# GuanLab/seekmer

Measured on AMD Instinct MI355X. Metric: paired reads/sec mapped+quantified, higher is better.
Workload: dtype u64+f64; 1 GPU; configs[1]: synthetic ~190k-tx index (stand-in for ENSEMBL GRCh38 cDNA), 10000000 2x100bp synthetic pairs per GPU, map+classes+EM to the reference stop rule; transcripts=190402, kmer_slots=134217728, units_per_gpu=10000000, read_len=100, paired=True, classes=851072, class_map_rows=4208693, parallelism=reads sharded x1, RCCL all-reduce f64[T] per EM step, rccl_ranks=0

## Files before the change

### seekmer_amd/csrc/skm_abi.hip

```cpp
#include "../../include/seekmer_hip.h"
#include "skm_kernels.h"
#include "skm_pool.h"

#include <dlfcn.h>
#include <algorithm>
#include <cstdarg>
#include <cstdio>
#include <cstdlib>
#include <cstring>
#include <chrono>
#include <condition_variable>
#include <atomic>
#include <deque>
#include <functional>
#include <map>
#include <memory>
#include <unordered_map>
#include <mutex>
#include <thread>
#include <numeric>
#include <string>
#include <utility>
#include <vector>

// ... 230 lines not shown
    PoolPinned pinned;
    std::mutex mu;
    int64_t n_tx = 0, n_classes = 0, n_ids = 0, n_rows = 0;
    DBuf<int64_t> cls_offset, row_start, tx_row;
    DBuf<int32_t> ids, tx_cls, row_tx, perm;
    DBuf<double> cls_count, cls_count_saved, inner, row_sum;
    DBuf<double> eff_len, x0, x1, acc, part_max;
    DBuf<unsigned int> part_flags, arrivals;
    DBuf<unsigned long long> ctl, cum;
    DBuf<unsigned int> tile_total;
    DBuf<double> x_start, boot_out;
    struct Batch {
        DBuf<double> cls_count, inner, row_sum, x0, x1, part_max;
        DBuf<unsigned int> part_flags;
        DBuf<unsigned long long> ctl, mgr;
        DBuf<double> counts_all;
        DBuf<double> totals;
        DBuf<int64_t> iters;
    } batch;
    struct Tiles {
        DBuf<int64_t> tile_tx, tile_cls, cls_pair, tx_pair;
        DBuf<int32_t> tx_list, cls_list, tx_label, tx_tile, cls_tile;
        DBuf<uint16_t> cls_tx, tx_cls;
        DBuf<double> snap, step_max;
        DBuf<unsigned int> step_flags;
        struct Residual {
            int64_t n_classes = 0, n_ids = 0, n_rows = 0;
            DBuf<int64_t> cls_offset, row_start, tx_row;
            DBuf<int32_t> ids, cls_src, row_tx, tx_cls;
            DBuf<double> cls_count, inner, row_sum;
            bool built = false;
        } residual;
        bool built = false;
        int64_t n_tiles = 0, n_oversize = 0;
    } tiles;
    double n_total = 0;
    bool n_total_reduced = false;
    void *comm = nullptr;
    int rank = 0, world = 1;
    double t_em_ns = 0, iters_total = 0, launches = 0;
};

struct skm_comm {
    int device = 0;
    void *comm = nullptr;
    int rank = 0, world = 1;
};

// ... 2341 lines not shown
    q->n_classes = n_classes;
    q->n_ids = n_ids;
    HIP_TRY(pool_stream_acquire(q->stream.out()));
    for (auto &e : q->ev) HIP_TRY(pool_event_acquire(e.out(), true));
    for (auto &e : q->chunk_ev) HIP_TRY(pool_event_acquire(e.out(), false));
    HIP_TRY(pool_pinned_acquire((void **)q->pinned.out()));
    const size_t C = (size_t)std::max<int64_t>(n_classes, 1), M = (size_t)std::max<int64_t>(n_ids, 1);
    const size_t T = (size_t)std::max<int64_t>(n_tx, 1);
    const size_t R = (size_t)quant_rows_upper_bound(n_tx, n_ids);
    SKM_TRY(q->cls_offset.ensure(C + 1));
    SKM_TRY(q->cls_count.ensure(C));
    SKM_TRY(q->inner.ensure(C));
    SKM_TRY(q->ids.ensure(M));
    SKM_TRY(q->perm.ensure(C));
    SKM_TRY(q->tx_cls.ensure(M));
    SKM_TRY(q->tx_row.ensure(T + 1));
    SKM_TRY(q->row_start.ensure(R + 1));
    SKM_TRY(q->row_tx.ensure(R));
    SKM_TRY(q->row_sum.ensure(R));
    SKM_TRY(q->eff_len.ensure(T));
    SKM_TRY(q->x0.ensure(T));
    SKM_TRY(q->x1.ensure(T));
    SKM_TRY(q->acc.ensure(T));
    SKM_TRY(q->ctl.ensure(16));
    SKM_TRY(q->part_max.ensure(EM_FINAL_BLOCKS));
    SKM_TRY(q->part_flags.ensure(EM_FINAL_BLOCKS));
    SKM_TRY(q->arrivals.ensure(T));
    HIP_TRY(hipMemsetAsync(q->arrivals.p, 0, T * sizeof(unsigned int), q->stream));
    if (em_tiles_possible(several_ranks)) {
        auto &t = q->tiles;
        SKM_TRY(t.tile_tx.ensure(T + 2)); SKM_TRY(t.tile_cls.ensure(T + 2));
        SKM_TRY(t.cls_pair.ensure(C + 1)); SKM_TRY(t.tx_pair.ensure(T + 1));
        SKM_TRY(t.tx_list.ensure(T)); SKM_TRY(t.cls_list.ensure(C));
        SKM_TRY(t.tx_label.ensure(T)); SKM_TRY(t.tx_tile.ensure(T)); SKM_TRY(t.cls_tile.ensure(C));
        SKM_TRY(t.cls_tx.ensure(M)); SKM_TRY(t.tx_cls.ensure(M));
    }
    STALE_CHECK("quant_alloc exit");
    return SKM_OK;
}

QuantBuild quant_build_view(skm_quant *q)
{
    QuantBuild b{};
    b.n_tx = q->n_tx;
    b.n_classes = q->n_classes;
    b.n_ids = q->n_ids;
    b.cls_offset = q->cls_offset.p;
// ... 8 lines not shown
        auto &t = q->tiles;
        b.tile_tx = t.tile_tx.p; b.tile_cls = t.tile_cls.p;
        b.tx_list = t.tx_list.p; b.cls_list = t.cls_list.p;
        b.cls_pair = t.cls_pair.p; b.tx_pair = t.tx_pair.p;
        b.tile_cls_tx = t.cls_tx.p; b.tile_tx_cls = t.tx_cls.p;
        b.tx_label = t.tx_label.p; b.tx_tile = t.tx_tile.p; b.cls_tile = t.cls_tile.p;
    }
    return b;
}

int quant_finish_setup(skm_quant *q, const ClassTable *table, int64_t units_seen = -1)
{
    STALE_CHECK("quant_finish_setup");
    QuantBuild b = quant_build_view(q);
    b.first_seen_bound = units_seen > 0 ? units_seen : 0;
    const int64_t rows = quant_setup(table, b, q->perm.p, q->stream);
    if (rows < 0) return fail(SKM_ERR_HIP, "building the class views failed (%lld): %s", (long long)rows, quant_setup_failure());
    q->n_rows = rows;
    if (b.tile_tx) {
        q->tiles.built = true;
        q->tiles.n_tiles = b.tile_info[0];
        q->tiles.n_oversize = b.tile_info[1];
        if (q->tiles.n_tiles > 0) {
            SKM_TRY(q->tiles.step_max.ensure((size_t)(EM_CHUNK_MAX * q->tiles.n_tiles)));
            SKM_TRY(q->tiles.step_flags.ensure((size_t)(EM_CHUNK_MAX * q->tiles.n_tiles)));
            SKM_TRY(q->tiles.snap.ensure((size_t)EM_CHUNK_MAX * (size_t)q->n_tx));
        }
        if (q->tiles.n_oversize > 0 && q->tiles.n_tiles > 0) {
            auto &r = q->tiles.residual;
            int64_t counts[3] = {0, 0, 0};
            if (quant_residual_count(b, counts, q->stream))
                return fail(SKM_ERR_HIP, "sizing the residual EM problem failed: %s", quant_setup_failure());
            r.n_classes = counts[0]; r.n_ids = counts[1]; r.n_rows = counts[2];
            SKM_TRY(r.cls_offset.ensure((size_t)r.n_classes + 1)); SKM_TRY(r.ids.ensure((size_t)std::max<int64_t>(r.n_ids, 1)));
            SKM_TRY(r.cls_src.ensure((size_t)std::max<int64_t>(r.n_classes, 1)));
            SKM_TRY(r.row_start.ensure((size_t)r.n_rows + 1)); SKM_TRY(r.row_tx.ensure((size_t)std::max<int64_t>(r.n_rows, 1)));
            SKM_TRY(r.tx_cls.ensure((size_t)std::max<int64_t>(r.n_ids, 1))); SKM_TRY(r.tx_row.ensure((size_t)q->n_tx + 1));
            SKM_TRY(r.cls_count.ensure((size_t)std::max<int64_t>(r.n_classes, 1)));
            SKM_TRY(r.inner.ensure((size_t)std::max<int64_t>(r.n_classes, 1)));
            SKM_TRY(r.row_sum.ensure((size_t)std::max<int64_t>(r.n_rows, 1)));
            QuantResidual out{};
            out.n_classes = r.n_classes; out.n_ids = r.n_ids; out.n_rows = r.n_rows;
            out.cls_offset = r.cls_offset.p; out.ids = r.ids.p; out.cls_src = r.cls_src.p;
            out.row_start = r.row_start.p; out.row_tx = r.row_tx.p; out.tx_cls = r.tx_cls.p; out.tx_row = r.tx_row.p;
            if (quant_residual_build(b, out, q->stream))
                return fail(SKM_ERR_HIP, "building the residual EM problem failed: %s", quant_setup_failure());
            r.built = true;
        }
// ... 98 lines not shown
        SKM_TRY(enqueue(slot));
        HIP_TRY(hipEventRecord(q->chunk_ev[slot], q->stream));
        return SKM_OK;
    };
    SKM_TRY(enqueue_chunk(0));
    for (int slot = 0;; slot ^= 1) {
        SKM_TRY(enqueue_chunk(slot ^ 1));
        HIP_TRY(hipEventSynchronize(q->chunk_ev[slot]));
        memcpy(words, q->pinned + 8 * slot, sizeof(words));
        if (stopped(words)) return SKM_OK;
    }
}
bool em_ctl_done(const unsigned long long *ctl) { return ctl[CTL_DONE] != 0; }

int em_run_tiles(skm_quant *q, const EmProblem &p, int64_t chunk, int64_t *iters_out)
{
    auto &t = q->tiles;
    EmTiles tl{};
    tl.n_tiles = t.n_tiles;
    tl.tile_tx = t.tile_tx.p; tl.tile_cls = t.tile_cls.p;
    tl.tx_list = t.tx_list.p; tl.cls_list = t.cls_list.p;
    tl.cls_pair = t.cls_pair.p; tl.tx_pair = t.tx_pair.p;
    tl.cls_tx = t.cls_tx.p; tl.tx_cls = t.tx_cls.p;
    tl.step_max = t.step_max.p; tl.step_flags = t.step_flags.p;
    tl.snap = t.snap.p;
    const bool mixed = t.n_oversize > 0;
    EmProblem pr = p;
    if (mixed) {
        auto &r = t.residual;
        pr.n_classes = r.n_classes; pr.n_rows = r.n_rows;
        pr.cls_offset = r.cls_offset.p; pr.ids = r.ids.p; pr.cls_count = r.cls_count.p; pr.inner = r.inner.p;
        pr.row_start = r.row_start.p; pr.row_tx = r.row_tx.p; pr.tx_cls = r.tx_cls.p; pr.tx_row = r.tx_row.p;
        pr.row_sum = r.row_sum.p;
        pr.fused = 1;
        pr.extra_max = t.step_max.p; pr.extra_flags = t.step_flags.p; pr.n_extra = t.n_tiles;
        launch_permute_f64(q->cls_count.p, r.cls_src.p, r.n_classes, r.cls_count.p, false, q->stream);
    }
    int64_t queued = 0;
    auto enqueue_chunk = [&](int slot) -> int {
        launch_em_local_chunk(p, tl, queued == 0 ? q->x0.p : t.snap.p + (chunk - 1) * q->n_tx, (int)chunk, queued * chunk, q->stream);
        if (mixed) {
            pr.extra_first = queued * chunk;
            for (int64_t i = 0, k = queued * chunk; i < chunk; ++i, ++k) {
                launch_em_inner(pr, (int)(k & 1), i > 0, k, q->stream);
                launch_em_rows_finalize(pr, (int)(k & 1), q->stream);
            }
            launch_em_decide(pr, (queued + 1) * chunk, q->stream);
            q->launches += 2 * chunk + 2;
        } else {
            launch_em_local_decide(p, tl, queued * chunk, (int)chunk, q->stream);
            q->launches += 2;
        }
        ++queued;
        HIP_TRY(hipGetLastError());
        HIP_TRY(hipMemcpyAsync(q->pinned + 8 * slot, q->ctl.p, 8 * sizeof(unsigned long long),
                               hipMemcpyDeviceToHost, q->stream));
        return SKM_OK;
    };
    unsigned long long ctl[8] = {0};
    SKM_TRY(em_run_chunks_ahead(q, ctl, enqueue_chunk, em_ctl_done));
    if (ctl[CTL_TILE_FAULT]) {
        HIP_TRY(hipStreamSynchronize(q->stream));
        return fail(SKM_ERR_STATE, "a component tile exceeds the tile capacity: the class views of this handle are damaged");
    }
    const int64_t steps = (int64_t)ctl[CTL_ITERS];
    HIP_TRY(hipEventRecord(q->ev[1], q->stream));
    HIP_TRY(hipEventSynchronize(q->ev[1]));
    float ms = 0;
    HIP_TRY(hipEventElapsedTime(&ms, q->ev[0], q->ev[1]));
    q->t_em_ns += ms * 1e6;
    q->iters_total += (double)steps;
    if (iters_out) *iters_out = steps;
    if (ctl[CTL_UNDEFINED]) return fail(SKM_ERR_UNDEFINED, "no abundance above x_floor: numpy raises on max() of an empty selection");
    return SKM_OK;
}

int em_run(skm_quant *q, double rel_tol, double x_floor, int64_t max_iters, int64_t fixed_iters,
           int64_t *iters_out, int64_t chunk_steps = 16)
{
    double n_total = q->n_total;
    if (q->comm && !q->n_total_reduced) {
        HIP_TRY(hipMemcpyAsync(q->acc.p, &n_total, 8, hipMemcpyHostToDevice, q->stream));
        NCCL_TRY(g_rccl.AllReduce(q->acc.p, q->acc.p, 1, NCCL_FLOAT64, NCCL_SUM, q->comm, q->stream));
        HIP_TRY(hipMemcpyAsync(&n_total, q->acc.p, 8, hipMemcpyDeviceToHost, q->stream));
        HIP_TRY(hipStreamSynchronize(q->stream));
    }
    EmProblem p = em_problem(q, rel_tol, x_floor, max_iters, fixed_iters);
    p.n_total = n_total;
    HIP_TRY(hipMemsetAsync(q->ctl.p, 0, 16 * 8, q->stream));
    int64_t k = 0;
    const int64_t chunk = fixed_iters > 0 ? std::min<int64_t>(fixed_iters, chunk_steps) : chunk_steps;
    HIP_TRY(hipEventRecord(q->ev[0], q->stream));
    if (em_uses_tiles(q) && chunk <= EM_CHUNK_MAX) return em_run_tiles(q, p, chunk, iters_out);
    static const bool unfused_rows = getenv("SKM_EM_UNFUSED") != nullptr;
    auto enqueue_chunk = [&](int slot) -> int {
        for (int64_t i = 0; i < chunk; ++i, ++k) {
            launch_em_inner(p, (int)(k & 1), i > 0, k, q->stream);
            if (q->comm) {
                if (unfused_rows) {
                    launch_em_rows(p, (int)(k & 1), q->stream);
                    launch_em_rows_to_acc(p, q->stream);
                } else {
                    launch_em_rows_acc(p, (int)(k & 1), q->stream);
                }
                NCCL_TRY(g_rccl.AllReduce(q->acc.p, q->acc.p, (size_t)q->n_tx, NCCL_FLOAT64, NCCL_SUM,
                                          q->comm, q->stream));
                launch_em_finalize(p, (int)(k & 1), true, q->stream);
            } else if (p.fused) {
                launch_em_rows_finalize(p, (int)(k & 1), q->stream);
            } else {
                launch_em_rows(p, (int)(k & 1), q->stream);
                launch_em_finalize(p, (int)(k & 1), false, q->stream);
// ... 210 lines not shown
    if (!q || !x || !l) return fail(SKM_ERR_ARG, "NULL argument");
    std::lock_guard<std::mutex> lock(q->mu);
    SKM_TRY(set_device(q->device));
    HIP_TRY(hipMemcpyAsync(q->x0.p, x, q->n_tx * 8, hipMemcpyHostToDevice, q->stream));
    HIP_TRY(hipMemcpyAsync(q->eff_len.p, l, q->n_tx * 8, hipMemcpyHostToDevice, q->stream));
    int64_t it = 0;
    SKM_TRY(em_run(q, rel_tol, x_floor, max_iters, fixed_iters, &it));
    HIP_TRY(hipMemcpy(x, (it & 1) ? q->x1.p : q->x0.p, q->n_tx * 8, hipMemcpyDeviceToHost));
    if (iters) *iters = it;
    return SKM_OK;
}

extern "C" int skm_quant_components(skm_quant *q, int64_t info[8], int32_t *tx_label, int32_t *tx_tile,
                                    int32_t *class_tile)
{
    if (!q || !info) return fail(SKM_ERR_ARG, "NULL argument");
    std::lock_guard<std::mutex> lock(q->mu);
    SKM_TRY(set_device(q->device));
    const auto &t = q->tiles;
    info[0] = t.built ? 1 : 0;
    info[1] = t.n_tiles;
    info[2] = t.n_oversize;
    info[3] = em_uses_tiles(q) ? 1 : 0;
    info[4] = EM_TILE_PAIRS; info[5] = EM_TILE_CLASSES; info[6] = EM_TILE_TX; info[7] = 0;
    if (!t.built) {
        if (tx_label || tx_tile || class_tile) return fail(SKM_ERR_ARG, "no component tiles were built for this handle");
        return SKM_OK;
    }
    HIP_TRY(hipStreamSynchronize(q->stream));
    if (tx_label) HIP_TRY(hipMemcpy(tx_label, t.tx_label.p, q->n_tx * 4, hipMemcpyDeviceToHost));
    if (tx_tile) HIP_TRY(hipMemcpy(tx_tile, t.tx_tile.p, q->n_tx * 4, hipMemcpyDeviceToHost));
    if (class_tile && q->n_classes) {
        std::vector<int32_t> tile(q->n_classes), perm(q->n_classes);
        HIP_TRY(hipMemcpy(tile.data(), t.cls_tile.p, q->n_classes * 4, hipMemcpyDeviceToHost));
        HIP_TRY(hipMemcpy(perm.data(), q->perm.p, q->n_classes * 4, hipMemcpyDeviceToHost));
        for (int64_t k = 0; k < q->n_classes; ++k) class_tile[perm[k]] = tile[k];
    }
    return SKM_OK;
}

extern "C" int skm_quant_set_counts(skm_quant *q, const double *class_counts)
{
    if (!q || (!class_counts && q->n_classes)) return fail(SKM_ERR_ARG, "NULL argument");
    std::lock_guard<std::mutex> lock(q->mu);
    SKM_TRY(set_device(q->device));
    const double total = np_sum_host(class_counts, q->n_classes);
    if (q->n_classes) {
// ... 845 lines not shown
```

### seekmer_amd/csrc/skm_em.hip

```cpp
#include "skm_em_core.h"

namespace skm {

__device__ bool em_evaluate(const EmProblem &p, int n_parts, int64_t steps_done, bool publish);

struct EmWholeTable {
    const EmProblem &p;
    __device__ __forceinline__ int64_t cls_first() const { return 0; }
    __device__ __forceinline__ int64_t cls_end() const { return p.n_classes; }
    __device__ __forceinline__ int64_t row_first() const { return 0; }
    __device__ __forceinline__ int64_t row_end() const { return p.n_rows; }
    __device__ __forceinline__ double n_total() const { return p.n_total; }
    __device__ __forceinline__ bool done() const { return p.ctl[CTL_DONE] != 0; }
    __device__ __forceinline__ bool judge(int eval_parts, int64_t steps_done) const { return em_evaluate(p, eval_parts, steps_done, true); }
    __device__ __forceinline__ int64_t part() const { return blockIdx.x; }
};

__global__ void __launch_bounds__(256)
em_inner_kernel(EmProblem p, int parity, int eval_parts, int64_t steps_done)
{
    em_inner_body(p, EmWholeTable{p}, parity, eval_parts > 0 && blockIdx.x == 0, eval_parts, steps_done, blockIdx.x * (int64_t)blockDim.x + threadIdx.x,
                  (int64_t)gridDim.x * blockDim.x);
}

// ... 110 lines not shown
    __shared__ uint16_t s_cls_tx[EM_TILE_PAIRS], s_tx_cls[EM_TILE_PAIRS];
    __shared__ uint16_t s_cls_off[EM_TILE_CLASSES + 1], s_tx_off[EM_TILE_TX + 1];
    const int64_t tile = blockIdx.x;
    const int64_t tx0 = tl.tile_tx[tile], cls0 = tl.tile_cls[tile];
    const int n_tx = (int)(tl.tile_tx[tile + 1] - tx0), n_cls = (int)(tl.tile_cls[tile + 1] - cls0);
    const int64_t cp0 = tl.cls_pair[cls0], tp0 = tl.tx_pair[tx0];
    const int n_pairs = (int)(tl.cls_pair[cls0 + n_cls] - cp0);
    if (n_tx > EM_TILE_TX || n_cls > EM_TILE_CLASSES || n_pairs > EM_TILE_PAIRS || n_tx < 0 || n_cls < 0 || n_pairs < 0) {
        if (threadIdx.x == 0) { p.ctl[CTL_TILE_FAULT] = 1; p.ctl[CTL_DONE] = 1; }
        return;
    }
    const int tid = threadIdx.x;
    if (p.ctl[CTL_DONE]) {
        const int64_t steps = (int64_t)p.ctl[CTL_ITERS], at = steps - 1 - (first_step - n_steps);
        if (p.ctl[CTL_TILE_FAULT] || first_step < n_steps || at < 0 || at >= n_steps) return;
        const double *__restrict__ from = tl.snap + at * p.n_tx;
        double *__restrict__ to = p.x[steps & 1];
        for (int i = tid; i < n_tx; i += 256) {
            const int32_t t = tl.tx_list[tx0 + i];
            to[t] = from[t];
        }
        return;
    }
    for (int j = tid; j < n_pairs; j += 256) {
        s_cls_tx[j] = tl.cls_tx[cp0 + j];
        s_tx_cls[j] = tl.tx_cls[tp0 + j];
    }
    for (int k = tid; k <= n_cls; k += 256) {
        s_cls_off[k] = (uint16_t)(tl.cls_pair[cls0 + k] - cp0);
        if (k < n_cls) s_count[k] = p.cls_count[tl.cls_list[cls0 + k]];
        if ((SKM_EM_TILE_EXPERIMENT & 1) && k < n_cls) s_inner[k] = 1.0;
    }
    for (int i = tid; i <= n_tx; i += 256) {
        s_tx_off[i] = (uint16_t)(tl.tx_pair[tx0 + i] - tp0);
        if (i < n_tx) {
            const int32_t t = tl.tx_list[tx0 + i];
            s_tx[i] = t;
            s_x[0][i] = x_in[t];
            s_eff[i] = p.eff_len[t];
        }
    }
    __syncthreads();
    const int sub = tid & 7, wave = tid >> 6;
    for (int step = 0; step < n_steps; ++step) {
        const double *x = s_x[step & 1];
        double *x_new = s_x[(step & 1) ^ 1];
// ... 35 lines not shown
                double a = 0.0;
                do {
                    const int row_end = min(begin + EM_ROW_CAP, end);
                    a += em_row_sum<false>(s_tx_cls, s_inner, begin, row_end, sub, xt);
                    begin = row_end;
                } while (begin < end);
                if (turn == sub) { my_a = a; my_xt = xt; my_i = i; }
            }
        }
        if (my_i >= 0) {
            const double v = em_new_abundance(my_a, s_eff[my_i], p.n_total);
            x_new[my_i] = v;
            tl.snap[step * p.n_tx + s_tx[my_i]] = v;
            em_note_change(v, my_xt, p.x_floor, local_max, flags);
        }
        em_wave_reduce<1>(local_max, flags);
        if ((tid & 63) == 0) { s_max[step][wave] = local_max; s_flags[step][wave] = flags; }
        __syncthreads();
    }
    if (tid < n_steps) {
        double m;
        unsigned int f;
        em_fold_waves(s_max[tid], s_flags[tid], 1, m, f);
        tl.step_max[tid * tl.n_tiles + tile] = m;
        tl.step_flags[tid * tl.n_tiles + tile] = f;
    }
}

__global__ void __launch_bounds__(64 * EM_CHUNK_MAX)
em_local_decide_kernel(EmProblem p, EmTiles tl, int64_t first_step, int n_steps)
{
    if (p.ctl[CTL_DONE]) return;
    __shared__ double s_max[EM_CHUNK_MAX];
    __shared__ unsigned int s_flags[EM_CHUNK_MAX];
    const int step = threadIdx.x >> 6, lane = threadIdx.x & 63;
    if (step < n_steps) {
        double m = 0.0;
        unsigned int f = 0;
        const double *__restrict__ step_max = tl.step_max + step * tl.n_tiles;
        const unsigned int *__restrict__ step_flags = tl.step_flags + step * tl.n_tiles;
        int64_t b = lane;
        for (; b + 7 * 64 < tl.n_tiles; b += 8 * 64) {
            double o[8];
            unsigned int g[8];
#pragma unroll
            for (int k = 0; k < 8; ++k) { o[k] = step_max[b + 64 * k]; g[k] = step_flags[b + 64 * k]; }
#pragma unroll
            for (int k = 0; k < 8; ++k) { m = o[k] > m ? o[k] : m; f |= g[k]; }
        }
        for (; b < tl.n_tiles; b += 64) {
            const double o = step_max[b];
            m = o > m ? o : m;
            f |= step_flags[b];
        }
        em_wave_reduce<1>(m, f);
        if (lane == 0) { s_max[step] = m; s_flags[step] = f; }
    }
    __syncthreads();
    if (threadIdx.x != 0) return;
    for (int s = 0; s < n_steps; ++s) {
        const int64_t steps_done = first_step + s + 1;
        const EmVerdict verdict = em_stop_rule(s_flags[s], s_max[s], p.rel_tol, steps_done, p.max_iters, p.fixed_iters);
        if (verdict.undefined) p.ctl[CTL_UNDEFINED] = 1;
        p.ctl[CTL_ITERS] = (unsigned long long)steps_done;
        p.ctl[CTL_DONE] = verdict.done ? 1ULL : 0ULL;
        if (verdict.done) break;
    }
}

__global__ void __launch_bounds__(256)
effective_lengths_kernel(const unsigned long long *__restrict__ fld,
                         const double *__restrict__ lengths, int64_t n_tx, double *__restrict__ out)
{
    fld += (int64_t)blockIdx.y * MAX_FRAGMENT_LENGTH;
    out += (int64_t)blockIdx.y * n_tx;
    __shared__ double p[MAX_FRAGMENT_LENGTH];
    __shared__ int bin[MAX_FRAGMENT_LENGTH];
    __shared__ unsigned long long counts[MAX_FRAGMENT_LENGTH];
    __shared__ unsigned long long part[4];
    __shared__ int n_bins;
    unsigned long long mine = 0;
    for (int i = threadIdx.x; i < MAX_FRAGMENT_LENGTH; i += blockDim.x) {
        counts[i] = fld[i];
        mine += counts[i];
    }
    for (int d = 32; d > 0; d >>= 1) mine += __shfl_xor(mine, d, 64);
    if ((threadIdx.x & 63) == 0) part[threadIdx.x >> 6] = mine;
    __syncthreads();
    const double total = (double)(long long)(part[0] + part[1] + part[2] + part[3]);
    if (threadIdx.x < 64) {
        int n = 0;
        for (int first = 0; first < MAX_FRAGMENT_LENGTH; first += 64) {
// ... 244 lines not shown

void launch_em_rows_finalize(const EmProblem &p, int parity, hipStream_t stream)
{
    hipLaunchKernelGGL(em_rows_finalize_kernel<false>, dim3((unsigned)em_final_blocks(p)), dim3(256), 0, stream, p, parity);
}

void launch_em_rows_acc(const EmProblem &p, int parity, hipStream_t stream)
{
    EmProblem fused = p;
    fused.fused = 1;
    hipLaunchKernelGGL(em_rows_finalize_kernel<true>, dim3((unsigned)em_final_blocks(fused)), dim3(256), 0, stream, p, parity);
}

void launch_em_local_chunk(const EmProblem &p, const EmTiles &tiles, const double *x_in, int n_steps, int64_t first_step,
                           hipStream_t stream)
{
    if (tiles.n_tiles <= 0 || n_steps <= 0) return;
    hipLaunchKernelGGL(em_local_chunk_kernel, dim3((unsigned)tiles.n_tiles), dim3(256), 0, stream, p, tiles, x_in,
                       std::min(n_steps, EM_CHUNK_MAX), first_step);
}

void launch_em_local_decide(const EmProblem &p, const EmTiles &tiles, int64_t first_step, int n_steps, hipStream_t stream)
{
    hipLaunchKernelGGL(em_local_decide_kernel, dim3(1), dim3(64 * EM_CHUNK_MAX), 0, stream, p, tiles, first_step,
                       std::min(n_steps, EM_CHUNK_MAX));
}

void launch_em_rows_to_acc(const EmProblem &p, hipStream_t stream)
{
    hipLaunchKernelGGL(em_rows_to_acc_kernel, dim3(chip_grid(p.n_tx, 256)), dim3(256), 0, stream, p);
}

void launch_em_finalize(const EmProblem &p, int parity, bool from_acc, hipStream_t stream)
{
    const int blocks = em_final_blocks(p);
    if (from_acc)
        hipLaunchKernelGGL(em_finalize_kernel<true>, dim3((unsigned)blocks), dim3(256), 0, stream, p, parity);
    else
        hipLaunchKernelGGL(em_finalize_kernel<false>, dim3((unsigned)blocks), dim3(256), 0, stream, p, parity);
}

constexpr int NP_MAX_LEAVES = 160;

__device__ __forceinline__ double np_leaf_sum(const double *a, int n)
{
    if (n < 8) {
        double r = 0.0;
// ... 289 lines not shown
```

### seekmer_amd/csrc/skm_kernels.h

```cpp
#pragma once
#include "skm_device.h"

namespace skm {

struct MapBatch {
    const uint32_t *records;
    int64_t n_units;
    int32_t words_per_read;
    int32_t record_words;
    int32_t paired;
    int32_t *workspace;
    int32_t *rec_unit;
    uint64_t *rec_key;
    unsigned long long *rec_tuple;
    int32_t keep_spans;
    int32_t *unit_begin, *unit_end;
    Coord *unit_anchor;
    int32_t *unit_entries;
    int64_t ids_capacity;
    unsigned long long *ids_cursor;
    unsigned long long *fld;
    unsigned long long *stats;
    int32_t vote[8];
};
// ... 143 lines not shown
    int fused;
    unsigned int *arrivals;
    const double *extra_max;
    const unsigned int *extra_flags;
    int64_t n_extra, extra_first;
};
enum { CTL_DONE = 0, CTL_ITERS = 1, CTL_UNDEFINED = 3, CTL_TILE_FAULT = 4 };
#ifndef SKM_EM_FINAL_BLOCKS
#define SKM_EM_FINAL_BLOCKS 2048
#endif
constexpr int EM_FINAL_BLOCKS = SKM_EM_FINAL_BLOCKS;
void launch_em_inner(const EmProblem &p, int parity, bool judge_previous, int64_t steps_done, hipStream_t stream);
void launch_em_decide(const EmProblem &p, int64_t steps_done, hipStream_t stream);
void launch_em_rows(const EmProblem &p, int parity, hipStream_t stream);
void launch_em_rows_finalize(const EmProblem &p, int parity, hipStream_t stream);
void launch_em_rows_acc(const EmProblem &p, int parity, hipStream_t stream);
void launch_em_rows_to_acc(const EmProblem &p, hipStream_t stream);
void launch_em_finalize(const EmProblem &p, int parity, bool from_acc, hipStream_t stream);
void launch_em_result(const unsigned long long *ctl, const double *x0, const double *x1, int64_t n, double *out,
                      hipStream_t stream);

constexpr int EM_TILE_PAIRS = 2048, EM_TILE_CLASSES = 512, EM_TILE_TX = 128;
#ifndef SKM_EM_TILE_SEGMENT
#define SKM_EM_TILE_SEGMENT 128
#endif
constexpr int EM_TILE_SEGMENT = SKM_EM_TILE_SEGMENT;
constexpr int EM_CHUNK_MAX = 16;
constexpr int EM_TILE_CLASS_BATCH = 4;
struct EmTiles {
    int64_t n_tiles;
    const int64_t *tile_tx;
    const int64_t *tile_cls;
    const int32_t *tx_list;
    const int32_t *cls_list;
    const int64_t *cls_pair;
    const int64_t *tx_pair;
    const uint16_t *cls_tx;
    const uint16_t *tx_cls;
    double *step_max;
    unsigned int *step_flags;
    double *snap;
};
void launch_em_local_chunk(const EmProblem &p, const EmTiles &tiles, const double *x_in, int n_steps, int64_t first_step,
                           hipStream_t stream);
void launch_em_local_decide(const EmProblem &p, const EmTiles &tiles, int64_t first_step, int n_steps, hipStream_t stream);

constexpr int EM_BATCH = 8;
struct EmBatchProblem {
    int64_t n_tx, n_classes, n_rows;
    const int64_t *cls_offset;
    const int32_t *ids;
    const int64_t *row_start;
    const int32_t *row_tx;
    const int32_t *tx_cls;
    const int64_t *tx_row;
    const double *eff_len;
    const double *cls_count;
    double *inner;
    double *row_sum;
    double *x[2];
    double *place_total;
    double rel_tol, x_floor;
    unsigned long long *ctl;
// ... 125 lines not shown
```

### seekmer_amd/csrc/skm_quant_setup.hip

```cpp
#include "skm_kernels.h"
#include "skm_pool.h"

#include <algorithm>
#include <cstdio>
#include <vector>

namespace skm {

namespace {

struct Scratch {
    hipStream_t stream;
    std::vector<void *> held;
    explicit Scratch(hipStream_t s) : stream(s) {}
    template <class T>
    T *alloc(size_t n)
    {
        void *p = nullptr;
        if (pool_alloc(&p, std::max<size_t>(n, 1) * sizeof(T)) != hipSuccess) return nullptr;
        held.push_back(p);
        return static_cast<T *>(p);
    }
    ~Scratch()
    {
// ... 705 lines not shown
__global__ void __launch_bounds__(256)
cc_classes_kernel(const int64_t *cls_offset, const int32_t *ids, int64_t n_classes, const int32_t *label,
                  int32_t *comp)
{
    const int lane = threadIdx.x & 63;
    const int64_t stride = (int64_t)gridDim.x * blockDim.x;
    for (int64_t c0 = blockIdx.x * (int64_t)blockDim.x + threadIdx.x - lane; c0 < n_classes; c0 += stride) {
        const int64_t c = c0 + lane;
        int32_t r = -1;
        if (c < n_classes) {
            const int64_t begin = cls_offset[c];
            r = label[begin < cls_offset[c + 1] ? ids[begin] : 0];
        }
        const int32_t before = __shfl_up(r, 1, 64);
        const unsigned long long heads = __ballot(lane == 0 || before != r);
        if (r >= 0 && ((heads >> lane) & 1ULL)) {
            const unsigned long long later = lane == 63 ? 0ULL : heads >> (lane + 1);
            const int run = later ? __ffsll((long long)later) : 64 - lane;
            atomicAdd(&comp[3 * (int64_t)r + 2], run);
        }
    }
}

__global__ void __launch_bounds__(256)
tile_pack_kernel(const int32_t *__restrict__ comp, int64_t n_tx, int64_t n_segments, int32_t *__restrict__ root_tile,
                 int64_t *__restrict__ seg_tiles, unsigned long long *__restrict__ oversize)
{
    for (int64_t g = blockIdx.x * (int64_t)blockDim.x + threadIdx.x; g < n_segments;
         g += (int64_t)gridDim.x * blockDim.x) {
        int tx = 0, pairs = 0, classes = 0, n = 0;
        const int64_t last = min(n_tx, (g + 1) * EM_TILE_SEGMENT);
        for (int64_t t0 = g * EM_TILE_SEGMENT; t0 < last; t0 += 8) {
            int size[24];
#pragma unroll
            for (int k = 0; k < 24; ++k) size[k] = 3 * t0 + k < 3 * n_tx ? comp[3 * t0 + k] : 0;
#pragma unroll
            for (int k = 0; k < 8; ++k) {
                const int64_t t = t0 + k;
                if (t >= last) break;
                const int c_tx = size[3 * k], c_pairs = size[3 * k + 1], c_classes = size[3 * k + 2];
                if (c_tx == 0) { root_tile[t] = -1; continue; }
                if (c_tx > EM_TILE_TX || c_pairs > EM_TILE_PAIRS || c_classes > EM_TILE_CLASSES) {
                    root_tile[t] = -2;
                    atomicAdd(oversize, 1ULL);
                    continue;
                }
                if (n == 0 || tx + c_tx > EM_TILE_TX || pairs + c_pairs > EM_TILE_PAIRS ||
                    classes + c_classes > EM_TILE_CLASSES) {
                    ++n;
                    tx = pairs = classes = 0;
                }
                tx += c_tx; pairs += c_pairs; classes += c_classes;
                root_tile[t] = n - 1;
            }
        }
        seg_tiles[g] = n;
    }
}

__global__ void __launch_bounds__(256)
tx_tile_kernel(const int32_t *label, const int32_t *root_tile, const int64_t *seg_base, int64_t n_tx,
               const int64_t *tx_row, const int64_t *row_start, int degree_bits, int32_t *tx_tile, int32_t *key)
{
    for (int64_t t = blockIdx.x * (int64_t)blockDim.x + threadIdx.x; t < n_tx;
         t += (int64_t)gridDim.x * blockDim.x) {
        const int32_t r = label[t], at = root_tile[r];
        const int32_t tile = at < 0 ? (int32_t)n_tx : (int32_t)(seg_base[r / EM_TILE_SEGMENT] + at);
        tx_tile[t] = tile;
        const int64_t turns = (row_start[tx_row[t + 1]] - row_start[tx_row[t]] + 7) >> 3;
        const int32_t longest = (1 << degree_bits) - 1;
        key[t] = (tile << degree_bits) | (longest - (int32_t)min(turns, (int64_t)longest));
    }
}

#ifndef SKM_EM_CLASS_ORDER
#define SKM_EM_CLASS_ORDER 1
#endif
__global__ void __launch_bounds__(256)
cls_tile_kernel(const int64_t *cls_offset, const int32_t *ids, int64_t n_classes, const int32_t *tx_tile,
                int length_bits, int32_t *cls_tile, int32_t *key)
{
// ... 73 lines not shown
    }
}

int build_tiles(Scratch &scratch, QuantBuild &q)
{
    hipStream_t stream = scratch.stream;
    const int64_t C = q.n_classes, M = q.n_ids, T = q.n_tx;
    if (M >= (1LL << 31) || C >= (1LL << 31) || T >= (1LL << 31) - 2) return -2;
    const int64_t n_segments = (T + EM_TILE_SEGMENT - 1) / EM_TILE_SEGMENT;
    QB_ALLOC(parent, int32_t, T); QB_ALLOC(comp, int32_t, 3 * T); QB_ALLOC(root_tile, int32_t, T);
    QB_ALLOC(seg_tiles, int64_t, n_segments); QB_ALLOC(seg_base, int64_t, n_segments + 1);
    QB_ALLOC(oversize, unsigned long long, 1);
    QB_ALLOC(iota, int32_t, std::max(T, C)); QB_ALLOC(sorted_tile, int32_t, std::max(T, C));
    QB_ALLOC(tx_local, int32_t, T); QB_ALLOC(cls_local, int32_t, C);
    QB_ALLOC(len, int64_t, std::max(T, C));
    QB_TRY(hipMemsetAsync(comp, 0, 3 * T * sizeof(int32_t), stream));
    QB_TRY(hipMemsetAsync(oversize, 0, sizeof(unsigned long long), stream));
    hipLaunchKernelGGL(iota_kernel, dim3(blocks_for(T)), dim3(256), 0, stream, parent, T);
    hipLaunchKernelGGL(cc_hook_kernel, dim3(blocks_for(C)), dim3(256), 0, stream, q.cls_offset, q.ids, C, parent);
    hipLaunchKernelGGL(cc_label_kernel, dim3(blocks_for(T)), dim3(256), 0, stream, parent, q.tx_row, q.row_start, T,
                       q.tx_label, comp);
    hipLaunchKernelGGL(cc_classes_kernel, dim3(blocks_for(C)), dim3(256), 0, stream, q.cls_offset, q.ids, C,
                       q.tx_label, comp);
    hipLaunchKernelGGL(tile_pack_kernel, dim3(blocks_for(n_segments)), dim3(256), 0, stream, comp, T, n_segments,
                       root_tile, seg_tiles, oversize);
    if (exclusive_scan_with_total(scratch, seg_tiles, seg_base, n_segments)) return -1;
    int end_bit = 1;
    while ((1LL << end_bit) < T + 1 && end_bit < 31) ++end_bit;
    const int degree_bits = end_bit + 5 <= 31 ? 5 : 0;
    QB_ALLOC(tx_key, int32_t, T);
    hipLaunchKernelGGL(tx_tile_kernel, dim3(blocks_for(T)), dim3(256), 0, stream, q.tx_label, root_tile, seg_base, T,
                       q.tx_row, q.row_start, degree_bits, q.tx_tile, tx_key);
    hipLaunchKernelGGL(iota_kernel, dim3(blocks_for(std::max(T, C))), dim3(256), 0, stream, iota, std::max(T, C));
    if (sort_pairs(scratch, tx_key, sorted_tile, iota, q.tx_list, T, end_bit + degree_bits)) return -1;
    hipLaunchKernelGGL(tile_starts_kernel, dim3(blocks_for(T + 1)), dim3(256), 0, stream, sorted_tile, degree_bits, T,
                       seg_base + n_segments, q.tile_tx);
    hipLaunchKernelGGL(tile_local_tx_kernel, dim3(blocks_for(T)), dim3(256), 0, stream, q.tx_list, sorted_tile, degree_bits,
                       q.tile_tx, seg_base + n_segments, T, q.tx_row, q.row_start, tx_local, len);
    if (exclusive_scan_with_total(scratch, len, q.tx_pair, T)) return -1;
    const int length_bits = SKM_EM_CLASS_ORDER ? degree_bits : 0;
    QB_ALLOC(cls_key, int32_t, C);
    hipLaunchKernelGGL(cls_tile_kernel, dim3(blocks_for(C)), dim3(256), 0, stream, q.cls_offset, q.ids, C, q.tx_tile,
                       length_bits, q.cls_tile, cls_key);
    if (sort_pairs(scratch, cls_key, sorted_tile, iota, q.cls_list, C, end_bit + length_bits)) return -1;
    hipLaunchKernelGGL(tile_starts_kernel, dim3(blocks_for(C + 1)), dim3(256), 0, stream, sorted_tile, length_bits, C,
                       seg_base + n_segments, q.tile_cls);
    hipLaunchKernelGGL(tile_local_cls_kernel, dim3(blocks_for(C)), dim3(256), 0, stream, q.cls_list, sorted_tile, length_bits,
// ... 160 lines not shown
```

### seekmer_amd/infer.py

```python
import ctypes
import datetime
import json
import logging
import os
import pathlib
import shlex
import sys

import numpy

from . import _native
from . import common
from . import mapper

__all__ = ['run', 'run_many', 'quantify', 'quantify_many', 'quantify_tables', 'quantify_resident', 'em', 'output_results', 'bootstrap_quantify',
           'bootstrap_ranks']

_LOG = logging.getLogger(__name__)

REL_TOL = 0.01
X_FLOOR = 1e-8


def run(index_path, output_path, fastq_paths, job_count, save_readmap,
# ... 271 lines not shown
        return cls(out, n_tx, offsets.size - 1)

    @classmethod
    def from_map_result(cls, map_result, n_tx):
        out = ctypes.c_void_p()
        _native.check(_native.hip().skm_quant_create_from_mapper(
            map_result._handle, n_tx, ctypes.byref(out)))
        return cls(out, n_tx, map_result.sizes()[0])

    def em(self, x, l, fixed_iters=0, max_iters=0, rel_tol=REL_TOL, x_floor=X_FLOOR):
        x = numpy.array(x, dtype='f8', copy=True, order='C')
        l = numpy.ascontiguousarray(l, dtype='f8')
        iters = ctypes.c_int64()
        _native.check(_native.hip().skm_quant_em(
            self.handle, _native.ptr(x, _native.c_f64p), _native.ptr(l, _native.c_f64p),
            rel_tol, x_floor, max_iters, fixed_iters, ctypes.byref(iters)))
        return x, iters.value

    def components(self, arrays=True):
        raw = numpy.zeros(8, dtype=numpy.int64)
        _native.check(_native.hip().skm_quant_components(self.handle, _native.ptr(raw, _native.c_i64p),
                                                         None, None, None))
        info = {'built': bool(raw[0]), 'tiles': int(raw[1]), 'oversize': int(raw[2]), 'em_uses_tiles': bool(raw[3]),
                'capacity': (int(raw[4]), int(raw[5]), int(raw[6]))}
        if not arrays or not info['built']:
            return info, None, None, None
        label = numpy.zeros(self.n_tx, dtype=numpy.int32)
        tile = numpy.zeros(self.n_tx, dtype=numpy.int32)
        class_tile = numpy.zeros(max(self.n_classes, 1), dtype=numpy.int32)
        _native.check(_native.hip().skm_quant_components(
            self.handle, _native.ptr(raw, _native.c_i64p), _native.ptr(label, _native.c_i32p),
            _native.ptr(tile, _native.c_i32p), _native.ptr(class_tile, _native.c_i32p)))
        return info, label, tile, class_tile[:self.n_classes]

    def set_counts(self, counts):
        counts = numpy.ascontiguousarray(counts, dtype='f8')
        _native.check(_native.hip().skm_quant_set_counts(self.handle,
                                                         _native.ptr(counts, _native.c_f64p)))

    def bootstrap(self, n_boot, seed, x0, l, want_counts=False, tpm=False):
        x0 = numpy.ascontiguousarray(x0, dtype='f8')
        l = numpy.ascontiguousarray(l, dtype='f8')
        out = numpy.zeros((n_boot, self.n_tx), dtype='f8')
        if tpm and not want_counts:
            iters = numpy.zeros(max(n_boot, 1), dtype=numpy.int64)
            _native.check(_native.hip().skm_quant_bootstrap_tpm(
                self.handle, n_boot, seed, _native.ptr(x0, _native.c_f64p),
# ... 413 lines not shown
```

Baseline: 969.0 million pairs/s.

## Fold per-tile EM convergence partials with atomics and pack tiles per wave

Each EM tile now folds its per-step max-change and flag partials straight into a small double-buffered area of the control words, using atomic max and or. This replaces the per-tile partial arrays that the decide kernel had to reduce, so the decide kernel shrinks to a single thread scanning at most 16 steps. Tile packing during setup now runs one wavefront per segment with ballot and shuffle instead of one thread per segment, and the segment run length doubles to 256. The price is atomic contention on a few global words, plus a change in tile packing that can alter tile counts.

```diff
diff --git a/seekmer_amd/csrc/skm_abi.hip b/seekmer_amd/csrc/skm_abi.hip
--- a/seekmer_amd/csrc/skm_abi.hip
+++ b/seekmer_amd/csrc/skm_abi.hip
@@ -276,8 +276,11 @@
         DBuf<int64_t> tile_tx, tile_cls, cls_pair, tx_pair;
         DBuf<int32_t> tx_list, cls_list, tx_label, tx_tile, cls_tile;
         DBuf<uint16_t> cls_tx, tx_cls;
-        DBuf<double> snap, step_max;
+        DBuf<double> snap;
+#if !SKM_EM_FOLD_PARTIALS
+        DBuf<double> step_max;
         DBuf<unsigned int> step_flags;
+#endif
         struct Residual {
             int64_t n_classes = 0, n_ids = 0, n_rows = 0;
             DBuf<int64_t> cls_offset, row_start, tx_row;
@@ -2665,7 +2668,7 @@
     SKM_TRY(q->x0.ensure(T));
     SKM_TRY(q->x1.ensure(T));
     SKM_TRY(q->acc.ensure(T));
-    SKM_TRY(q->ctl.ensure(16));
+    SKM_TRY(q->ctl.ensure(16 + EM_FOLD_WORDS));
     SKM_TRY(q->part_max.ensure(EM_FINAL_BLOCKS));
     SKM_TRY(q->part_flags.ensure(EM_FINAL_BLOCKS));
     SKM_TRY(q->arrivals.ensure(T));
@@ -2720,8 +2723,10 @@
         q->tiles.n_tiles = b.tile_info[0];
         q->tiles.n_oversize = b.tile_info[1];
         if (q->tiles.n_tiles > 0) {
+#if !SKM_EM_FOLD_PARTIALS
             SKM_TRY(q->tiles.step_max.ensure((size_t)(EM_CHUNK_MAX * q->tiles.n_tiles)));
             SKM_TRY(q->tiles.step_flags.ensure((size_t)(EM_CHUNK_MAX * q->tiles.n_tiles)));
+#endif
             SKM_TRY(q->tiles.snap.ensure((size_t)EM_CHUNK_MAX * (size_t)q->n_tx));
         }
         if (q->tiles.n_oversize > 0 && q->tiles.n_tiles > 0) {
@@ -2866,7 +2871,12 @@
     tl.tx_list = t.tx_list.p; tl.cls_list = t.cls_list.p;
     tl.cls_pair = t.cls_pair.p; tl.tx_pair = t.tx_pair.p;
     tl.cls_tx = t.cls_tx.p; tl.tx_cls = t.tx_cls.p;
+#if SKM_EM_FOLD_PARTIALS
+    tl.step_max = reinterpret_cast<double *>(q->ctl.p + 16);
+    tl.step_flags = reinterpret_cast<unsigned int *>(q->ctl.p + 16 + 2 * EM_CHUNK_MAX);
+#else
     tl.step_max = t.step_max.p; tl.step_flags = t.step_flags.p;
+#endif
     tl.snap = t.snap.p;
     const bool mixed = t.n_oversize > 0;
     EmProblem pr = p;
@@ -2877,7 +2887,7 @@
         pr.row_start = r.row_start.p; pr.row_tx = r.row_tx.p; pr.tx_cls = r.tx_cls.p; pr.tx_row = r.tx_row.p;
         pr.row_sum = r.row_sum.p;
         pr.fused = 1;
-        pr.extra_max = t.step_max.p; pr.extra_flags = t.step_flags.p; pr.n_extra = t.n_tiles;
+        pr.extra_max = tl.step_max; pr.extra_flags = tl.step_flags; pr.n_extra = SKM_EM_FOLD_PARTIALS ? 1 : t.n_tiles;
         launch_permute_f64(q->cls_count.p, r.cls_src.p, r.n_classes, r.cls_count.p, false, q->stream);
     }
     int64_t queued = 0;
@@ -2885,6 +2895,10 @@
         launch_em_local_chunk(p, tl, queued == 0 ? q->x0.p : t.snap.p + (chunk - 1) * q->n_tx, (int)chunk, queued * chunk, q->stream);
         if (mixed) {
             pr.extra_first = queued * chunk;
+#if SKM_EM_FOLD_PARTIALS
+            pr.extra_max = tl.step_max + (queued & 1) * EM_CHUNK_MAX;
+            pr.extra_flags = tl.step_flags + (queued & 1) * EM_CHUNK_MAX;
+#endif
             for (int64_t i = 0, k = queued * chunk; i < chunk; ++i, ++k) {
                 launch_em_inner(pr, (int)(k & 1), i > 0, k, q->stream);
                 launch_em_rows_finalize(pr, (int)(k & 1), q->stream);
@@ -2931,7 +2945,7 @@
     }
     EmProblem p = em_problem(q, rel_tol, x_floor, max_iters, fixed_iters);
     p.n_total = n_total;
-    HIP_TRY(hipMemsetAsync(q->ctl.p, 0, 16 * 8, q->stream));
+    HIP_TRY(hipMemsetAsync(q->ctl.p, 0, (16 + EM_FOLD_WORDS) * 8, q->stream));
     int64_t k = 0;
     const int64_t chunk = fixed_iters > 0 ? std::min<int64_t>(fixed_iters, chunk_steps) : chunk_steps;
     HIP_TRY(hipEventRecord(q->ev[0], q->stream));
@@ -3188,7 +3202,7 @@
     info[1] = t.n_tiles;
     info[2] = t.n_oversize;
     info[3] = em_uses_tiles(q) ? 1 : 0;
-    info[4] = EM_TILE_PAIRS; info[5] = EM_TILE_CLASSES; info[6] = EM_TILE_TX; info[7] = 0;
+    info[4] = EM_TILE_PAIRS; info[5] = EM_TILE_CLASSES; info[6] = EM_TILE_TX; info[7] = EM_TILE_SEGMENT;
     if (!t.built) {
         if (tx_label || tx_tile || class_tile) return fail(SKM_ERR_ARG, "no component tiles were built for this handle");
         return SKM_OK;
diff --git a/seekmer_amd/csrc/skm_em.hip b/seekmer_amd/csrc/skm_em.hip
--- a/seekmer_amd/csrc/skm_em.hip
+++ b/seekmer_amd/csrc/skm_em.hip
@@ -156,6 +156,13 @@
         }
         return;
     }
+#if SKM_EM_FOLD_PARTIALS
+    const int fold = (int)((first_step / n_steps) & 1) * EM_CHUNK_MAX;
+    if (tile == 0 && tid < EM_CHUNK_MAX) {
+        tl.step_max[(fold ^ EM_CHUNK_MAX) + tid] = 0.0;
+        tl.step_flags[(fold ^ EM_CHUNK_MAX) + tid] = 0u;
+    }
+#endif
     for (int j = tid; j < n_pairs; j += 256) {
         s_cls_tx[j] = tl.cls_tx[cp0 + j];
         s_tx_cls[j] = tl.tx_cls[tp0 + j];
@@ -237,11 +244,47 @@
         double m;
         unsigned int f;
         em_fold_waves(s_max[tid], s_flags[tid], 1, m, f);
+#if SKM_EM_FOLD_PARTIALS
+        const unsigned long long bits = (unsigned long long)__double_as_longlong(m);
+        if (bits)
+            (void)__hip_atomic_fetch_max(reinterpret_cast<unsigned long long *>(tl.step_max) + fold + tid, bits,
+                                         __ATOMIC_RELAXED, __HIP_MEMORY_SCOPE_AGENT);
+        if (f)
+            (void)__hip_atomic_fetch_or(tl.step_flags + fold + tid, f, __ATOMIC_RELAXED, __HIP_MEMORY_SCOPE_AGENT);
+#else
         tl.step_max[tid * tl.n_tiles + tile] = m;
         tl.step_flags[tid * tl.n_tiles + tile] = f;
-    }
-}
-
+#endif
+    }
+}
+
+#if SKM_EM_FOLD_PARTIALS
+__global__ void __launch_bounds__(64)
+em_local_decide_kernel(EmProblem p, EmTiles tl, int64_t first_step, int n_steps)
+{
+    if (p.ctl[CTL_DONE]) return;
+    if (threadIdx.x != 0) return;
+    const int fold = (int)((first_step / n_steps) & 1) * EM_CHUNK_MAX;
+    double m[EM_CHUNK_MAX];
+    unsigned int f[EM_CHUNK_MAX];
+#pragma unroll
+    for (int s = 0; s < EM_CHUNK_MAX; ++s) {
+        m[s] = s < n_steps ? tl.step_max[fold + s] : 0.0;
+        f[s] = s < n_steps ? tl.step_flags[fold + s] : 0u;
+    }
+    bool stopped = false;
+#pragma unroll
+    for (int s = 0; s < EM_CHUNK_MAX; ++s) {
+        if (s >= n_steps || stopped) continue;
+        const int64_t steps_done = first_step + s + 1;
+        const EmVerdict verdict = em_stop_rule(f[s], m[s], p.rel_tol, steps_done, p.max_iters, p.fixed_iters);
+        if (verdict.undefined) p.ctl[CTL_UNDEFINED] = 1;
+        p.ctl[CTL_ITERS] = (unsigned long long)steps_done;
+        p.ctl[CTL_DONE] = verdict.done ? 1ULL : 0ULL;
+        stopped = verdict.done;
+    }
+}
+#else
 __global__ void __launch_bounds__(64 * EM_CHUNK_MAX)
 em_local_decide_kernel(EmProblem p, EmTiles tl, int64_t first_step, int n_steps)
 {
@@ -283,6 +326,8 @@
     }
 }
 
+#endif
+
 __global__ void __launch_bounds__(256)
 effective_lengths_kernel(const unsigned long long *__restrict__ fld,
                          const double *__restrict__ lengths, int64_t n_tx, double *__restrict__ out)
@@ -573,7 +618,7 @@
 
 void launch_em_local_decide(const EmProblem &p, const EmTiles &tiles, int64_t first_step, int n_steps, hipStream_t stream)
 {
-    hipLaunchKernelGGL(em_local_decide_kernel, dim3(1), dim3(64 * EM_CHUNK_MAX), 0, stream, p, tiles, first_step,
+    hipLaunchKernelGGL(em_local_decide_kernel, dim3(1), dim3(SKM_EM_FOLD_PARTIALS ? 64 : 64 * EM_CHUNK_MAX), 0, stream, p, tiles, first_step,
                        std::min(n_steps, EM_CHUNK_MAX));
 }
 
diff --git a/seekmer_amd/csrc/skm_kernels.h b/seekmer_amd/csrc/skm_kernels.h
--- a/seekmer_amd/csrc/skm_kernels.h
+++ b/seekmer_amd/csrc/skm_kernels.h
@@ -189,10 +189,14 @@
 
 constexpr int EM_TILE_PAIRS = 2048, EM_TILE_CLASSES = 512, EM_TILE_TX = 128;
 #ifndef SKM_EM_TILE_SEGMENT
-#define SKM_EM_TILE_SEGMENT 128
+#define SKM_EM_TILE_SEGMENT 256
 #endif
 constexpr int EM_TILE_SEGMENT = SKM_EM_TILE_SEGMENT;
 constexpr int EM_CHUNK_MAX = 16;
+#ifndef SKM_EM_FOLD_PARTIALS
+#define SKM_EM_FOLD_PARTIALS 1
+#endif
+constexpr int EM_FOLD_WORDS = SKM_EM_FOLD_PARTIALS ? 2 * EM_CHUNK_MAX + EM_CHUNK_MAX : 0;
 constexpr int EM_TILE_CLASS_BATCH = 4;
 struct EmTiles {
     int64_t n_tiles;
@@ -204,8 +208,13 @@
     const int64_t *tx_pair;
     const uint16_t *cls_tx;
     const uint16_t *tx_cls;
+#if SKM_EM_FOLD_PARTIALS
     double *step_max;
     unsigned int *step_flags;
+#else
+    double *step_max;
+    unsigned int *step_flags;
+#endif
     double *snap;
 };
 void launch_em_local_chunk(const EmProblem &p, const EmTiles &tiles, const double *x_in, int n_steps, int64_t first_step,
diff --git a/seekmer_amd/csrc/skm_quant_setup.hip b/seekmer_amd/csrc/skm_quant_setup.hip
--- a/seekmer_amd/csrc/skm_quant_setup.hip
+++ b/seekmer_amd/csrc/skm_quant_setup.hip
@@ -751,6 +751,52 @@
     }
 }
 
+#ifndef SKM_TILE_PACK_WAVE
+#define SKM_TILE_PACK_WAVE 1
+#endif
+static_assert(EM_TILE_SEGMENT >= 64 && EM_TILE_SEGMENT <= 1024 && (EM_TILE_SEGMENT & (EM_TILE_SEGMENT - 1)) == 0,
+              "tile_pack_kernel takes a run 64 ids at a time: a power of two from 64 to 1024");
+#if SKM_TILE_PACK_WAVE
+constexpr int TILE_PACK_LANES = 64;
+__global__ void __launch_bounds__(256)
+tile_pack_kernel(const int32_t *__restrict__ comp, int64_t n_tx, int64_t n_segments, int32_t *__restrict__ root_tile,
+                 int64_t *__restrict__ seg_tiles, unsigned long long *__restrict__ oversize)
+{
+    const int lane = threadIdx.x & 63;
+    const int64_t n_waves = ((int64_t)gridDim.x * blockDim.x) >> 6;
+    unsigned long long above = 0;
+    for (int64_t g = (blockIdx.x * (int64_t)blockDim.x + threadIdx.x) >> 6; g < n_segments; g += n_waves) {
+        int tx = 0, pairs = 0, classes = 0, n = 0;
+        const int64_t last = min(n_tx, (g + 1) * EM_TILE_SEGMENT);
+        for (int64_t t0 = g * EM_TILE_SEGMENT; t0 < last; t0 += 64) {
+            const int64_t t = t0 + lane;
+            int c_tx = 0, c_pairs = 0, c_classes = 0;
+            if (t < last) { c_tx = comp[3 * t]; c_pairs = comp[3 * t + 1]; c_classes = comp[3 * t + 2]; }
+            const bool root = c_tx != 0;
+            const bool alone = root && (c_tx > EM_TILE_TX || c_pairs > EM_TILE_PAIRS || c_classes > EM_TILE_CLASSES);
+            above += (unsigned long long)__popcll(__ballot(alone));
+            int32_t mine = alone ? -2 : -1;
+            unsigned long long todo = __ballot(root && !alone);
+            while (todo) {
+                const int at = __ffsll((long long)todo) - 1;
+                todo &= todo - 1;
+                const int r_tx = __shfl(c_tx, at, 64), r_pairs = __shfl(c_pairs, at, 64), r_classes = __shfl(c_classes, at, 64);
+                if (n == 0 || tx + r_tx > EM_TILE_TX || pairs + r_pairs > EM_TILE_PAIRS ||
+                    classes + r_classes > EM_TILE_CLASSES) {
+                    ++n;
+                    tx = pairs = classes = 0;
+                }
+                tx += r_tx; pairs += r_pairs; classes += r_classes;
+                if (lane == at) mine = n - 1;
+            }
+            if (t < last) root_tile[t] = mine;
+        }
+        if (lane == 0) seg_tiles[g] = n;
+    }
+    if (lane == 0 && above) atomicAdd(oversize, above);
+}
+#else
+constexpr int TILE_PACK_LANES = 1;
 __global__ void __launch_bounds__(256)
 tile_pack_kernel(const int32_t *__restrict__ comp, int64_t n_tx, int64_t n_segments, int32_t *__restrict__ root_tile,
                  int64_t *__restrict__ seg_tiles, unsigned long long *__restrict__ oversize)
@@ -786,6 +832,7 @@
         seg_tiles[g] = n;
     }
 }
+#endif
 
 __global__ void __launch_bounds__(256)
 tx_tile_kernel(const int32_t *label, const int32_t *root_tile, const int64_t *seg_base, int64_t n_tx,
@@ -905,7 +952,7 @@
                        q.tx_label, comp);
     hipLaunchKernelGGL(cc_classes_kernel, dim3(blocks_for(C)), dim3(256), 0, stream, q.cls_offset, q.ids, C,
                        q.tx_label, comp);
-    hipLaunchKernelGGL(tile_pack_kernel, dim3(blocks_for(n_segments)), dim3(256), 0, stream, comp, T, n_segments,
+    hipLaunchKernelGGL(tile_pack_kernel, dim3(blocks_for(n_segments * TILE_PACK_LANES)), dim3(256), 0, stream, comp, T, n_segments,
                        root_tile, seg_tiles, oversize);
     if (exclusive_scan_with_total(scratch, seg_tiles, seg_base, n_segments)) return -1;
     int end_bit = 1;
diff --git a/seekmer_amd/infer.py b/seekmer_amd/infer.py
--- a/seekmer_amd/infer.py
+++ b/seekmer_amd/infer.py
@@ -317,7 +317,7 @@
         _native.check(_native.hip().skm_quant_components(self.handle, _native.ptr(raw, _native.c_i64p),
                                                          None, None, None))
         info = {'built': bool(raw[0]), 'tiles': int(raw[1]), 'oversize': int(raw[2]), 'em_uses_tiles': bool(raw[3]),
-                'capacity': (int(raw[4]), int(raw[5]), int(raw[6]))}
+                'capacity': (int(raw[4]), int(raw[5]), int(raw[6])), 'run': int(raw[7])}
         if not arrays or not info['built']:
             return info, None, None, None
         label = numpy.zeros(self.n_tx, dtype=numpy.int32)
```

New measurement: 1.003 billion pairs/s, median of 6. +3.5%, better.
